# fallenshock/SinDDM

Measured on AMD Instinct MI355X. Metric: diffusion steps/sec (finest scale) + imgs/sec full multi-scale sample, 1/2/4/8 GPU, higher is better.
Workload: dtype f32 (3x3 convs: binary16 hi/lo split products -- Winograd-domain GEMMs with all 4 MFMA terms, fp32 accumulate; fp32-equivalent, error vs float64 = the fp32 oracle's: tests/test_gpu_h2.py; everything else fp32); 1 GPU; C3: 6-scale pyramid, T=1000, finest scale 411x512, batch 64 per GPU, dim=160; batch_per_gpu=64, global_batch=64, scale=5, parallelism=independent chains over 1 GPU(s), one all-gather of the images

## Files before the change

### include/sinddm_hip_debug.h

```cpp
#ifndef SINDDM_HIP_DEBUG_H
#define SINDDM_HIP_DEBUG_H

#include <stddef.h>
#include <stdint.h>

#ifdef __cplusplus
extern "C" {
#endif

int sinddm_prof_begin(void);
int sinddm_prof_end(double* conv_ms_total, int64_t* conv_launches, double* conv_flops_total);
int sinddm_prof_end2(double* conv_ms_total, int64_t* conv_launches, double* conv_flops_total,
                     double* conv_exec_flops_total);
int sinddm_prof_end3(int kind, double* ms_total, int64_t* launches, double* flops_total,
                     double* exec_flops_total, int reset);

int sinddm_debug_routes(int dim_arg, int train, int B, int H, int W, int out[16]);

int sinddm_debug_conv_path(int dim, int B, int H, int W);

int sinddm_debug_infer_path(int dim, int B, int H, int W);

int sinddm_debug_head_path(int dim, int B, int H, int W);
int sinddm_debug_head_offsets(int dim, int64_t out[3]);
int sinddm_debug_head(const float* packed, const float* g, const float* x_in, float* eps_out, int dim, int B, int H, int W,
                      int Wp, void* stream);

int sinddm_debug_train_path(int dim, int B, int H, int W);

int sinddm_debug_block_train(const float* params, const float* packed, const float* packed_bwd, int dim, int l,
                             const float* x, const float* cond_bias, const float* grad_y, float* y, float* grad_x,
                             float* grad_params, float* dcond, int B, int H, int W, void* ws, size_t ws_bytes,
                             void* stream);

int sinddm_debug_wgrad_map(int Cin, int Cout, int64_t ntiles, int ncu, uint32_t* wg_out, int wg_cap, int32_t* splits_out,
                           int splits_cap);

#define SINDDM_DWGRAD_TILES 6
#define SINDDM_DWGRAD_ROWS 7
int sinddm_debug_wgrad_plan(int taps, int Cin, int Cout, int B, int H, int W, int have_scr, int have_amax, int ncu, int out[4]);
int sinddm_debug_wgrad(int taps, int Cin, int Cout, int B, int H, int W, int ncu, int have_scr, int use_amax, const float* dout,
                       const float* in, float* gw, float* gb, void* scratch, size_t scratch_bytes, int plan_out[4], void* stream);
size_t sinddm_debug_wgrad_scratch_bytes(int taps, int Cin, int Cout, int B);
int sinddm_debug_wgrad_routes(int dim_arg, int B, int H, int W, int ncu, int* out, int cap);
// ... 6 lines not shown
```

### sinddm_amd/_lib.py

```python
from __future__ import annotations

import ctypes as C
import os
from typing import Optional

import torch

_HERE = os.path.dirname(os.path.abspath(__file__))
LIB_PATH = os.path.join(_HERE, "libsinddm_hip.so")

ABI_SYMBOLS = (
    "sinddm_abi_version", "sinddm_param_count", "sinddm_param_tensors", "sinddm_param_offset",
    "sinddm_packed_count", "sinddm_workspace_bytes", "sinddm_pack_weights", "sinddm_net_forward",
    "sinddm_q_sample", "sinddm_reverse_step", "sinddm_reverse_step_edit", "sinddm_upsample_bilinear", "sinddm_prof_begin", "sinddm_prof_end", "sinddm_prof_end2", "sinddm_prof_end3", "sinddm_debug_wgrad_map", "sinddm_debug_conv_path",
    "sinddm_debug_block_train", "sinddm_debug_infer_path", "sinddm_debug_train_path",
    "sinddm_train_workspace_bytes", "sinddm_packed_bwd_count", "sinddm_pack_weights_bwd",
    "sinddm_net_forward_train", "sinddm_net_backward", "sinddm_l1_loss_fwd_bwd", "sinddm_adam_ema_step",
    "sinddm_cond_embed", "sinddm_cond_stride", "sinddm_sample_chain", "sinddm_sample_chain2", "sinddm_sample_chain_ex",
    "sinddm_normal_fill", "sinddm_wrap_halo", "sinddm_upsample_bilinear_wrap", "sinddm_sample_chain_tile",
    "sinddm_sample_chain_keep", "sinddm_reverse_step_keep", "sinddm_normal_fill_samples", "sinddm_sample_chain_seeds",
    "sinddm_debug_head_path", "sinddm_debug_head_offsets", "sinddm_debug_head", "sinddm_debug_routes",
    "sinddm_debug_wgrad_routes", "sinddm_debug_wgrad_plan", "sinddm_debug_wgrad", "sinddm_debug_wgrad_scratch_bytes",
    "sinddm_sample_chain_resample", "sinddm_reverse_step_jump",
    "sinddm_sample_chain_layout", "sinddm_layout_delta", "sinddm_reverse_step_layout",
    "sinddm_sample_chain_batch",
    "sinddm_sample_chain_solver", "sinddm_reverse_step_ms",
    "sinddm_q_sample_wrap", "sinddm_l1_loss_crop_fwd_bwd",
    "sinddm_sample_chain_mix", "sinddm_normal_fill_mix",
    "sinddm_l1_loss_weighted_fwd_bwd",
)


ABI_VERSION = 3
DIM_FP32_CONVS = 0x10000
JUMP_STREAM = 1 << 31
MIX_MAX = 4
TILE_HALO = 16


class StepCoefs(C.Structure):
    _fields_ = [("mode", C.c_int), ("clip", C.c_int),
                ("sqrt_recip_ac_t", C.c_float), ("sqrt_recipm1_ac_t", C.c_float),
                ("coef1_t", C.c_float), ("coef2_t", C.c_float),
                ("gamma_t", C.c_float), ("gamma_tm1", C.c_float),
# ... 108 lines not shown
        "sinddm_prof_end": (i, [C.POINTER(C.c_double), C.POINTER(C.c_int64), C.POINTER(C.c_double)]),
        "sinddm_prof_end2": (i, [C.POINTER(C.c_double), C.POINTER(C.c_int64), C.POINTER(C.c_double),
                                 C.POINTER(C.c_double)]),
        "sinddm_prof_end3": (i, [i, C.POINTER(C.c_double), C.POINTER(C.c_int64), C.POINTER(C.c_double),
                                 C.POINTER(C.c_double), i]),
        "sinddm_debug_wgrad_map": (i, [i, i, i64, i, C.POINTER(C.c_uint32), i, C.POINTER(C.c_int32), i]),
        "sinddm_debug_conv_path": (i, [i, i, i, i]),
        "sinddm_debug_infer_path": (i, [i, i, i, i]),
        "sinddm_debug_train_path": (i, [i, i, i, i]),
        "sinddm_debug_head_path": (i, [i, i, i, i]),
        "sinddm_debug_routes": (i, [i, i, i, i, i, C.POINTER(C.c_int)]),
        "sinddm_debug_wgrad_routes": (i, [i, i, i, i, i, C.POINTER(C.c_int), i]),
        "sinddm_debug_wgrad_plan": (i, [i, i, i, i, i, i, i, i, i, C.POINTER(C.c_int)]),
        "sinddm_debug_wgrad": (i, [i, i, i, i, i, i, i, i, i, p, p, p, p, p, sz, C.POINTER(C.c_int), p]),
        "sinddm_debug_wgrad_scratch_bytes": (sz, [i, i, i, i]),
        "sinddm_debug_head_offsets": (i, [i, C.POINTER(C.c_int64)]),
        "sinddm_debug_head": (i, [p, p, p, p, i, i, i, i, i, p]),
        "sinddm_debug_block_train": (i, [p, p, p, i, i, p, p, p, p, p, p, p, i, i, i, p, sz, p]),
        "sinddm_train_workspace_bytes": (sz, [i, i, i, i]),
        "sinddm_packed_bwd_count": (i64, [i]),
        "sinddm_pack_weights_bwd": (i, [p, p, i, p]),
        "sinddm_net_forward_train": (i, [p, p, p, p, i, f, p, i, i, i, i, p, sz, p]),
        "sinddm_net_backward": (i, [p, p, p, p, p, p, p, i, i, i, i, p, sz, p]),
        "sinddm_l1_loss_fwd_bwd": (i, [p, p, p, p, i64, f, p]),
        "sinddm_l1_loss_crop_fwd_bwd": (i, [p, p, p, p, i, i, i, i, i, f, p]),
        "sinddm_l1_loss_weighted_fwd_bwd": (i, [p, p, p, p, p, i, i, i, i, i, i, f, f, p]),
        "sinddm_adam_ema_step": (i, [p, p, p, p, p, f, f, f, f, f, f, f, i, i64, p]),
    }
    for name, (res, args) in sig.items():
        if not hasattr(lib, name):
# ... 32 lines not shown
```

### sinddm_amd/csrc/conv_wh.h

```cpp
#pragma once
#include <utility>
#include "split16.h"

namespace sinddm {

template <class F, int... I>
__device__ __forceinline__ void wh_static_for_impl(F&& f, std::integer_sequence<int, I...>) {
    (f(std::integral_constant<int, I>{}), ...);
}
template <int N, class F>
__device__ __forceinline__ void wh_static_for(F&& f) {
    wh_static_for_impl(f, std::make_integer_sequence<int, N>{});
}

#ifndef WH_ABL
#define WH_ABL 0
#endif
#ifndef WH_MIXLO
#define WH_MIXLO 1
#endif
#ifndef WH_NT
#define WH_NT 6
#endif
#ifdef WH_TIMING
// ... 3 lines not shown
#define WH_SEG(slot) do {} while (0)
#endif
constexpr int WH_TH = 8, WH_TW = 32;
constexpr int WH_RS = 40;
constexpr int WH_PS = 408;
constexpr int WH_RAW = 16 * WH_PS * 4;
constexpr int WH_V = 24 * 2 * 64 * 16;
constexpr int WH_XS = 36;
constexpr int WH_X = 2 * 6 * 32 * WH_XS * 4;
constexpr int WH_LDS = 160 * 1024;
constexpr int WH_REGION = WH_LDS - WH_RAW;
constexpr int WH_VB = WH_REGION - WH_V;
static_assert(WH_X <= WH_VB && WH_V + WH_X <= WH_REGION && WH_VB % 16 == 0, "exchange buffer beside either V buffer");
constexpr int WH_TARGET_EXP = 10;
constexpr int WH_COB = 80;

inline bool wh_shape_ok(int cin, int cout) { return cin >= 32 && cin % 16 == 0 && cout % WH_COB == 0; }
inline long long wh_image_halfs(int cin, int cout) { return (long long)(cout / WH_COB) * (cin / 16) * 24 * 5 * 512; }

__device__ __forceinline__ int wh_shift_for(float m, int target) {
    const unsigned bits = __float_as_uint(m) & 0x7fffffffu;
    const int e = (int)(bits >> 23);
    if (e == 0 || e == 255) return 0;
    int s = target - (e - 127);
    return s > 100 ? 100 : (s < -100 ? -100 : s);
}

__device__ __forceinline__ void wh_u24(const float* __restrict__ w, long long base, int transpose, double (&u)[24]) {
    const double G2[4][3] = {{1., 0., 0.}, {.5, .5, .5}, {.5, -.5, .5}, {0., 0., 1.}};
    const double G4[6][3] = {{1. / 4, 0., 0.}, {-1. / 6, -1. / 6, -1. / 6}, {-1. / 6, 1. / 6, -1. / 6},
// ... 84 lines not shown
    hipLaunchKernelGGL(wh_pack_kernel, dim3((unsigned)((total + 255) / 256)), dim3(256), 0, st, w, wsinv,
                       static_cast<_Float16*>(img), cin, cout, transpose, total);
    SINDDM_LAUNCH_CHECK();
    return 0;
}

__device__ __forceinline__ void wh_barrier() { asm volatile("s_waitcnt lgkmcnt(0)\n\ts_barrier" ::: "memory"); }

__device__ __forceinline__ float wh_dpp_shr2(float old, float src) {
    return __builtin_bit_cast(float, __builtin_amdgcn_update_dpp(__builtin_bit_cast(int, old), __builtin_bit_cast(int, src), 0x112, 0xf, 0xf, false));
}
__device__ __forceinline__ float wh_dpp_shl2(float old, float src) {
    return __builtin_bit_cast(float, __builtin_amdgcn_update_dpp(__builtin_bit_cast(int, old), __builtin_bit_cast(int, src), 0x102, 0xf, 0xf, false));
}

__global__ __launch_bounds__(512) void conv_wh_kernel(ConvArgs p, int items_per_xcd, int wg_per_xcd) {
    typedef __attribute__((address_space(3))) float lds_f;
    extern __shared__ __attribute__((aligned(16))) float smem[];
    unsigned char* const sbytes = reinterpret_cast<unsigned char*>(smem);
    unsigned char* const sRaw = sbytes;
    unsigned char* const sV = sbytes + WH_RAW;
    const unsigned lds0 = (unsigned)(size_t)(lds_f*)smem;

    const int tid = threadIdx.x;
    const int lane = tid & 63;
    const int wv = __builtin_amdgcn_readfirstlane(tid >> 6);
    const int l16 = lane & 15, kq = lane >> 4;
    const int H = p.H, W = p.W;
    const int HW = H * W;
    const int Wt = p.Wt > 0 ? p.Wt : W;
    const int nch = p.nch3;
// ... 134 lines not shown
#else
                        const f32x2 rem{__builtin_fmaf(v[j].x, sxv, -(float)hi[pr][j].x), __builtin_fmaf(v[j].y, sxv, -(float)hi[pr][j].y)};
                        lo[pr][j] = __builtin_convertvector(rem, h16x2);
#endif
                    }
                }
#pragma unroll
                for (int j = 0; j < 6; ++j) {
                    using h16x4 = __attribute__((ext_vector_type(4))) _Float16;
                    *reinterpret_cast<h16x4*>(wp + (i * 6 + j) * 2048) = h16x4{hi[0][j][0], hi[0][j][1], hi[1][j][0], hi[1][j][1]};
                    *reinterpret_cast<h16x4*>(wp + (i * 6 + j) * 2048 + 512) = h16x4{lo[0][j][0], lo[0][j][1], lo[1][j][0], lo[1][j][1]};
                }
            });
        };

        f32x4 acc[4][2][5];
#pragma unroll
        for (int a = 0; a < 4; ++a)
#pragma unroll
            for (int g = 0; g < 2; ++g)
#pragma unroll
                for (int n = 0; n < 5; ++n) acc[a][g][n] = f32x4{0.f, 0.f, 0.f, 0.f};
        const __amdgpu_buffer_rsrc_t rsw =
            __builtin_amdgcn_make_buffer_rsrc(const_cast<float*>(p.w3), 0, 0x7FFFFFF0, 0x00020000);
        const int wlane = lane * 16;
        const int wbase = ((cb * nch) * 24 + fj) * 5 * 1024;
        h16x8 ur[10];
        auto load_u = [&](int c, int fi, int n, int slot) {
            const int so = wbase + (c * 24 * 5 + fi * 30 + n) * 1024;
            ur[slot] = __builtin_bit_cast(h16x8, __builtin_amdgcn_raw_buffer_load_b128(rsw, wlane, so, 0));
        };
        auto multiply = [&](int c, const unsigned char* vb) {
            const unsigned char* A = vb + fj * 2048 + a_rd;
            wh_static_for<4>([&](auto FI) {
                constexpr int fi = decltype(FI)::value;
                constexpr int fo = fi * 6 * 2048;
                h16x8 ah0, ah1, al0, al1;
                ah0 = *reinterpret_cast<const h16x8*>(A + fo);
                ah1 = *reinterpret_cast<const h16x8*>(A + fo + 1024);
                al0 = *reinterpret_cast<const h16x8*>(A + fo + 512);
                al1 = *reinterpret_cast<const h16x8*>(A + fo + 1024 + 512);
                wh_static_for<5>([&](auto NN) {
                    constexpr int n = decltype(NN)::value;
                    constexpr int slot = (fi & 1) * 5 + n;
                    const h16x8 u = ur[slot];
                    __builtin_amdgcn_sched_barrier(0);
                    if (WH_ABL & 8) {
// ... 2 lines not shown
                        acc[fi][0][n] = __builtin_amdgcn_mfma_f32_16x16x32_f16(al0, u, acc[fi][0][n], 0, 0, 0);
                        acc[fi][1][n] = __builtin_amdgcn_mfma_f32_16x16x32_f16(al1, u, acc[fi][1][n], 0, 0, 0);
                        acc[fi][0][n] = __builtin_amdgcn_mfma_f32_16x16x32_f16(ah0, u, acc[fi][0][n], 0, 0, 0);
                        acc[fi][1][n] = __builtin_amdgcn_mfma_f32_16x16x32_f16(ah1, u, acc[fi][1][n], 0, 0, 0);
                    }
                    __builtin_amdgcn_sched_barrier(0);
                    if (!(WH_ABL & 4)) {
                        if (fi < 2) load_u(c, fi + 2, n, slot);
                        else load_u(c + 1 < nch ? c + 1 : c, fi - 2, n, slot);
                    }
                    __builtin_amdgcn_sched_barrier(0);
                });
            });
        };

        const int e_t = tid & 31, e_co = tid >> 5;
        const int e_tr = e_t >> 3, e_tc = e_t & 7;
        const int ey = y0 + 2 * e_tr, ex = x0 + 4 * e_tc;
        f32x4 rsd[5][2];
        float ek[5], ebv[5];
        auto ep_operands = [&]() {
            const bool e_in = ex < W;
#pragma unroll
            for (int n = 0; n < 5; ++n) {
                const int co = cb * WH_COB + n * 16 + e_co;
                ek[n] = inv_sx * p.wsinv[co];
                ebv[n] = p.bias ? p.bias[co] : 0.0f;
#pragma unroll
                for (int pp = 0; pp < 2; ++pp) {
                    rsd[n][pp] = f32x4{0.f, 0.f, 0.f, 0.f};
                    if (p.resid && !(WH_ABL & 16) && e_in && ey + pp < H)
                        rsd[n][pp] = ((WH_NT & 2) && big_out) ? __builtin_nontemporal_load(reinterpret_cast<const f32x4*>(p.resid + ((size_t)b * p.Cout + co) * HW + (size_t)(ey + pp) * W + ex))
                                                 : *reinterpret_cast<const f32x4*>(p.resid + ((size_t)b * p.Cout + co) * HW + (size_t)(ey + pp) * W + ex);
                }
            }
        };

        WH_SEG(0);
        if constexpr (service) {
            const __amdgpu_buffer_rsrc_t rsnx = in_rsrc(nxt.ok ? nxt.b : b);
            float sxn = 0.f, inv_n = 0.f;
            if (nxt.ok) item_scale(nxt, sxn, inv_n);
            if (j == 0) {
                stage_write(sRaw);
                if (nch > 1) stage_load(rsin, svoff, 1);
                else if (nxt.ok) { stage_offsets(nxt, svoff); stage_load(rsnx, svoff, 0); }
                WH_SEG(1);
                transform(sRaw, vbuf(g), sx);
                wh_barrier();
            }
            WH_SEG(2);
            for (int c = 0; c < nch; ++c) {
                if (c + 1 < nch || nxt.ok) {
                    stage_write(sRaw);
                    if (c + 2 < nch) stage_load(rsin, svoff, c + 2);
                    else if (nxt.ok) {
                        if (c + 2 == nch) stage_offsets(nxt, svoff);
                        if (c + 2 == nch || nch > 1) stage_load(rsnx, svoff, c + 2 - nch);
                    }
                    if (c == 3) WH_SEG(24);
                    transform(sRaw, vbuf(g + c + 1), c + 1 < nch ? sx : sxn);
                    if (c == 3) WH_SEG(25);
                }
                wh_barrier();
                if (c < 12) WH_SEG(3 + c);
            }
            ep_operands();
        } else {
            wh_static_for<10>([&](auto SL) {
                constexpr int sl = decltype(SL)::value;
                load_u(0, sl / 5, sl % 5, sl);
            });
            WH_SEG(1);
            if (j == 0) wh_barrier();
            WH_SEG(2);
            for (int c = 0; c < nch; ++c) {
                multiply(c, vbuf(g + c));
                if (c == 3) WH_SEG(25);
                wh_barrier();
                if (c < 12) WH_SEG(3 + c);
            }
            ep_operands();
        }
        g += nch;
        WH_SEG(16);

        const int e_wr = ((fj * 32 + l16) * WH_XS + 4 * kq) * 4;
        const int e_rd = (e_co * WH_XS + e_t) * 4;
        float amax = 0.f;
        WH_SEG(17);
        if constexpr (!service) {
#pragma unroll
            for (int mg = 0; mg < 2; ++mg)
#pragma unroll
                for (int n = 0; n < 5; ++n) {
                    acc[0][mg][n] = acc[0][mg][n] + acc[1][mg][n] + acc[2][mg][n];
                    acc[1][mg][n] = acc[1][mg][n] - acc[2][mg][n] - acc[3][mg][n];
                }
        }
        wh_static_for<3>([&](auto PS) {
            constexpr int n0 = 2 * decltype(PS)::value;
            constexpr int nn = n0 + 2 <= 5 ? 2 : 1;
            unsigned char* X = sV + ((g & 1) ? 0 : WH_V);
            if constexpr (!service) {
#pragma unroll
                for (int r = 0; r < 2; ++r)
#pragma unroll
                    for (int nl = 0; nl < nn; ++nl)
#pragma unroll
                        for (int mg = 0; mg < 2; ++mg)
                            *reinterpret_cast<f32x4*>(X + e_wr + (r * 6 * 32 + nl * 16) * (WH_XS * 4) + mg * 64) = acc[r][mg][n0 + nl];
            }
            wh_barrier();
            WH_SEG(18 + decltype(PS)::value);
            float q[nn][2][6];
#pragma unroll
            for (int nl = 0; nl < nn; ++nl)
#pragma unroll
                for (int r = 0; r < 2; ++r)
#pragma unroll
                    for (int j = 0; j < 6; ++j)
                        q[nl][r][j] = *reinterpret_cast<const float*>(X + e_rd + ((r * 6 + j) * 32 + nl * 16) * (WH_XS * 4));
            wh_barrier();
            wh_static_for<nn>([&](auto NL) {
                constexpr int n = n0 + decltype(NL)::value;
                const int co = cb * WH_COB + n * 16 + e_co;
                const float k = ek[n];
                const float bv = ebv[n];
#pragma unroll
                for (int pp = 0; pp < 2; ++pp) {
                    const float* z = q[decltype(NL)::value][pp];
                    const float s12 = z[1] + z[2], d12 = z[1] - z[2], s34 = z[3] + z[4], d34 = z[3] - z[4];
                    f32x4 v{z[0] + s12 + s34, d12 + 2.f * d34, s12 + 4.f * s34, d12 + 8.f * d34 + z[5]};
                    const int y = ey + pp;
                    if ((WH_ABL & 16) && v[0] != 123.456f) continue;
                    if (y < H && ex < W) {
                        const size_t o = ((size_t)b * p.Cout + co) * HW + (size_t)y * W + ex;
                        v = v * k + bv;
                        if (p.out_pre) *reinterpret_cast<f32x4*>(p.out_pre + o) = v;
                        if (p.act == 1) v = gelu_erf4(v);
                        else if (p.act == 2) {
// ... 12 lines not shown
                        else *reinterpret_cast<f32x4*>(p.out + o) = v;
                    }
                }
            });
        });
        if (p.amax_out) amax_publish(amax, p.amax_out + (size_t)b * AMAX_STRIDE);
        WH_SEG(23);
        if (!nxt.ok) break;
        cur = nxt;
    }
    };
    if (service_rt) role_body(std::true_type{});
    else role_body(std::false_type{});
}

#ifndef SINDDM_WH_MIN_ITEMS_PER_CU
#define SINDDM_WH_MIN_ITEMS_PER_CU 12
#endif
#ifndef SINDDM_WH_MIN_PIXELS
#define SINDDM_WH_MIN_PIXELS 12000
#endif
#ifndef SINDDM_CONV_WH
#define SINDDM_CONV_WH 1
#endif
inline bool conv_wh_applies(bool fp32_convs, int B, int H, int W, int cin, int cout) {
    if (!SINDDM_CONV_WH || fp32_convs || !wh_shape_ok(cin, cout) || W % 4 != 0) return false;
    if ((long long)cin * H * W * 4 >= 0x40000000LL) return false;
    if ((long long)H * W < SINDDM_WH_MIN_PIXELS) return false;
    return (long long)B * ((W + WH_TW - 1) / WH_TW) * ((H + WH_TH - 1) / WH_TH) * (cout / WH_COB) >=
           (long long)SINDDM_WH_MIN_ITEMS_PER_CU * cu_count();
}

inline int conv_wh_launch(const ConvArgs& a_in, hipStream_t st) {
    ConvArgs a = a_in;
    if (!wh_shape_ok(a.Cin, a.Cout) || a.W % 4 != 0 || !a.wsinv || (long long)a.Cin * a.H * a.W * 4 >= 0x40000000LL)
        return SINDDM_E_BADSHAPE;
    ConvProfiler& prof = conv_profiler();
    const bool rec = prof.begin(st);
    a.nch3 = a.Cin / 16;
    a.coblks = a.Cout / WH_COB;
    a.tilesX = (a.W + WH_TW - 1) / WH_TW;
    a.tilesY = (a.H + WH_TH - 1) / WH_TH;
    a.ntiles = a.B * a.tilesX * a.tilesY;
    a.tiles_per_xcd = (a.ntiles + 7) / 8;
    const int ipx = a.tiles_per_xcd * a.coblks;
    int wpx = cu_count() / 8;
    if (wpx < 1) wpx = 1;
    if (wpx > ipx) wpx = ipx;
    static const hipError_t attr_rc = hipFuncSetAttribute(reinterpret_cast<const void*>(&conv_wh_kernel),
                                                          hipFuncAttributeMaxDynamicSharedMemorySize, WH_LDS);
    if (attr_rc != hipSuccess) return (int)attr_rc;
#ifdef WH_TIMING
    static int wh_launch_no = 0;
    a.mtp = wh_launch_no++ % 8;
#endif
    hipLaunchKernelGGL(conv_wh_kernel, dim3(wpx * 8), dim3(512), WH_LDS, st, a, ipx, wpx);
    if (rec) {
        const double fl = 2.0 * a.B * a.H * (a.Wt > 0 ? a.Wt : a.W) * (double)a.Cout * 9.0 * a.Cin;
        prof.end(st, 1, fl, 2.0 * a.ntiles * 32.0 * 24.0 * 4.0 * (double)a.Cout * a.Cin, 8);
    }
    SINDDM_LAUNCH_CHECK();
    return 0;
}

}
```

### sinddm_amd/csrc/internal.h

```cpp
#pragma once
#include "common.h"

namespace sinddm {

struct PackSeg {
    long long dst;
    long long count;
    long long w;
    long long w2;
    int kind;
    int cin, cout, taps, nch, mt, co_lds;
    int transpose;
};
struct PackArgs {
    PackSeg seg[32];
    int nseg;
    long long total;
};
int pack_launch(const float* params, float* packed, const PackArgs& a, hipStream_t st);

inline void pack_add_direct(PackArgs& a, long long dst, long long w, int cin, int cout, int taps, int mt, int coblks, int transpose) {
    PackSeg s{};
    s.kind = 0; s.transpose = transpose; s.w2 = -1;
    s.dst = dst; s.w = w; s.cin = cin; s.cout = cout; s.taps = taps; s.mt = mt; s.co_lds = co_lds_for(mt);
// ... 35 lines not shown
    float* wscr;
    float* amax;
};

struct ChainStep;
int net_forward_impl(const NetPlan& P, const float* params, const float* packed, const float* x, const int64_t* t_dev,
                     int t_host, float scale, float* out, int B, int H, int W, void* ws, size_t ws_bytes,
                     hipStream_t st, const TrainBufs* tb, const ChainStep* cs = nullptr);

int block_forward(const NetPlan& P, int l, const float* params, const float* packed, const float* cur, const float* cond,
                  int cond_stride, float* hbuf, float* gbuf, float* obuf, float* upre, int B, int H, int W, hipStream_t st,
                  const int route[2], int Wt = 0, float* amax = nullptr);
enum ConvKernel { CONV_DIRECT = 0, CONV_C3 = 1, CONV_WINO2 = 2, CONV_WINO3 = 3, CONV_WINO4 = 4, CONV_WH = 8 };
ConvKernel conv3x3_route(const NetPlan& P, const Conv3x3Images& c, int B, int H, int W, bool have_amax, bool first_conv);
struct ConvArgs;
int conv3x3_launch(ConvKernel k, const Conv3x3Images& c, const float* packed, ConvArgs a, hipStream_t st);
bool forward_routes(const NetPlan& P, bool train, int B, int H, int Wp, bool have_amax, int out[8]);
int forward_pitch(const NetPlan& P, int W);

bool wh_enabled();
int wh_pack(const Conv3x3Images& c, const float* w, float* packed, int transpose, hipStream_t st);
int amax_tensor_launch(const float* x, float* amax, int B, long long per_sample, hipStream_t st);

int dwconv_launch(const float* x, const float* w, const float* bias, const float* cond, int cond_stride,
                  const float* addt, int flip, float* out, int B, int C, int H, int W, hipStream_t st, int pi = 0, int po = 0,
                  float* amax = nullptr);

}
```

### sinddm_amd/csrc/sinddm_bwd.hip

```cpp
#include <utility>
#include "conv_args.h"
#include "conv1x1.h"
#include "internal.h"
#include "wgrad_plan.h"
#include "wgrad_wh.h"

namespace sinddm {

struct WgradArgs {
    const float* dout;
    const float* in;
    const float* zero;
    float* gw;
    float* gb;
    int B, H, W, Cin, Cout;
    int coblks, ciblks, S;
    int tilesX, tilesY, ntiles;
    int abl;
    int scr;
};

template <int MT, int TAPS>
__global__ __launch_bounds__(WG_THREADS, 2) void wgrad_mfma_kernel(WgradArgs p) {
    typedef __attribute__((address_space(3))) void* lds_ptr;
// ... 966 lines not shown
        rc = amax_tensor_launch(dO, amax_b + 2 * l, B, (long long)b.cout * H * W, st);
        if (rc) return rc;
    }
    rc = wgrad_launch(d.w2, zp, dO, tb.g[l], grads + b.c2_w, grads + b.c2_b, st, tb.wscr, d.wh2 ? amax_b + 2 * l : nullptr,
                      d.wh2 ? tb.amax + 2 * l + 1 : nullptr);
    if (rc) return rc;
    if (d.wres.nwg > 0) {
        rc = wgrad_launch(d.wres, zp, dO, xin, grads + b.res_w, grads + b.res_b, st);
        if (rc) return rc;
    }
    {
        ConvArgs c{};
        c.zero = zp; c.in = dO; c.Cin = b.cout; c.aux = tb.u[l]; c.act = 2; c.out = dU; c.Cout = b.cout;
        c.B = B; c.H = H; c.W = W;
        if (d.wh2) { c.amax_in = amax_b + 2 * l; c.amax_out = d.wh1 ? amax_b + 2 * l + 1 : nullptr; }
        rc = conv3x3_launch(d.dg2, k.dg2[l], packed_bwd, c, st);
    }
    if (rc) return rc;
    rc = wgrad_launch(d.w1, zp, dU, tb.h[l], grads + b.c1_w, grads + b.c1_b, st, tb.wscr, d.wha ? amax_b + 2 * l + 1 : nullptr,
                      d.wha ? tb.amax + 2 * l : nullptr);
    if (rc) return rc;
    {
        ConvArgs c{};
        c.zero = zp; c.in = dU; c.Cin = b.cout; c.act = 0; c.out = dH; c.Cout = b.cin;
        c.B = B; c.H = H; c.W = W;
        if (d.wh1) c.amax_in = amax_b + 2 * l + 1;
        rc = conv3x3_launch(d.dg1, k.dg1[l], packed_bwd, c, st);
    }
    if (rc) return rc;
    hipLaunchKernelGGL(d.dw_rows ? dwconv5_wgrad_rows_kernel : dwconv5_wgrad_kernel, dim3(b.cin, B), dim3(256), 0, st, dH, xin,
                       grads + b.dw_w, grads + b.dw_b, tb.dcond + b.cond_off, P.cond_stride, b.cin, H, W);
    SINDDM_LAUNCH_CHECK();
    if (dst) {
        const float* radd = dO;
        if (b.res_w >= 0) {
            rc = conv1x1_dgrad(zp, dO, b.cout, packed_bwd + k.dres[l], conv3x3_nch(k.dg1[l]), dU, b.cin, k.dg1[l].mt,
                               k.dg1[l].coblks, B, H, W, st);
            if (rc) return rc;
            radd = dU;
        }
        rc = dwconv_launch(dH, params + b.dw_w, nullptr, nullptr, 0, radd, 1, dst, B, b.cin, H, W, st, 0, 0,
                           d.pub ? amax_b + 2 * (l - 1) : nullptr);
// ... 309 lines not shown
```

### sinddm_amd/csrc/sinddm_fwd.hip

```cpp
#include "conv_mfma.h"
#include "conv_wino4.h"
#include "conv_wh.h"
#include "internal.h"
#include "step_tail.h"
#include "chain_run.h"
#include <type_traits>
namespace sinddm {

ConvProfiler& conv_profiler() {
    static ConvProfiler p;
    return p;
}

__global__ void pack_kernel(const float* __restrict__ params, float* __restrict__ packed, PackArgs a) {
    long long i = (long long)blockIdx.x * blockDim.x + threadIdx.x;
    if (i >= a.total) return;
    int s = 0;
    long long base = 0;
    while (s < a.nseg - 1 && i >= base + a.seg[s].count) { base += a.seg[s].count; ++s; }
    const PackSeg& g = a.seg[s];
    const long long j = i - base;
    float v = 0.0f;
    if (g.kind == 0) {
        const int co_l = (int)(j % g.co_lds);
// ... 813 lines not shown
static HeadEps head_eps(const NetPlan& P, const float* packed, const float* g, const float* xin, int H, int Wp) {
    return HeadEps{g, xin, packed + P.pk_hc, packed + P.pk_hr, packed + P.pk_hb, P.half, P.dim, H, Wp};
}

ConvKernel conv3x3_route(const NetPlan& P, const Conv3x3Images& c, int B, int H, int W, bool have_amax, bool first_conv) {
    if (wino_enabled() && c.K % 4 == 0) {
        if (have_amax && c.wh >= 0 && conv_wh_applies(P.fp32_convs, B, H, W, c.K, c.M)) return CONV_WH;
        if (SINDDM_WINO_V3 && c.wino24 >= 0 &&
            (long long)B * ((W + 31) / 32) * ((H + 3) / 4) * c.coblks >= SINDDM_V3_MIN_ITEMS_PER_CU * cu_count())
            return SINDDM_WINO_V4 && conv_wino4_applies(B, H, W, c.coblks) ? CONV_WINO4 : CONV_WINO3;
        if (c.wino2 >= 0) return CONV_WINO2;
    }
    return first_conv && c.K == 3 && SINDDM_CONV_C3 ? CONV_C3 : CONV_DIRECT;
}

int conv3x3_launch(ConvKernel k, const Conv3x3Images& c, const float* packed, ConvArgs a, hipStream_t st) {
    a.coblks = c.coblks;
    switch (k) {
        case CONV_WH:
            a.w3 = packed + c.wh; a.wsinv = packed + c.wh_sinv;
            return conv_wh_launch(a, st);
        case CONV_WINO4:
        case CONV_WINO3:
            a.w3 = packed + c.wino24; a.nch3 = conv3x3_nchw(c);
            return k == CONV_WINO4 ? conv_wino4_launch(a, st) : conv_wino3_launch(a, st);
        case CONV_WINO2:
            if (a.Cin % 4 != 0) return SINDDM_E_BADSHAPE;
            a.w3 = packed + c.wino2; a.nch3 = conv3x3_nchw(c);
            return conv_wino2_launch(a, c.mt, st);
        case CONV_DIRECT:
            a.w3 = packed + c.direct; a.nch3 = conv3x3_nch(c);
            return conv_launch(a, c.mt, st);
        default: return SINDDM_E_BADARG;
    }
}

// ... 3 lines not shown
    for (int l = 0; l < 4; ++l) {
        out[2 * l] = conv3x3_route(P, P.blk[l].c1, B, H, Wp, have_amax, true);
        out[2 * l + 1] = head && l == 3 ? -1 : conv3x3_route(P, P.blk[l].c2, B, H, Wp, have_amax, false);
        any = any || out[2 * l] == CONV_WH || out[2 * l + 1] == CONV_WH;
    }
    return any;
}
int forward_pitch(const NetPlan& P, int W) { return fwd_pitch(P, W); }

int block_forward(const NetPlan& P, int l, const float* params, const float* packed, const float* cur, const float* cond,
                  int cond_stride, float* hbuf, float* gbuf, float* obuf, float* upre, int B, int H, int W, hipStream_t st,
                  const int route[2], int Wt, float* amax) {
    const BlockPlan& b = P.blk[l];
    const bool wha = route[0] == CONV_WH, whb = route[1] == CONV_WH;
    if ((wha || whb) && !amax) return SINDDM_E_BADARG;
    int rc = Wt > 0 ? dwconv_launch(cur, params + b.dw_w, params + b.dw_b, cond, cond_stride, nullptr, 0, hbuf, B, b.cin, H,
                                    Wt, st, W, W, wha ? amax : nullptr)
                    : dwconv_launch(cur, params + b.dw_w, params + b.dw_b, cond, cond_stride, nullptr, 0, hbuf, B, b.cin, H,
                                    W, st, 0, 0, wha ? amax : nullptr);
    if (rc) return rc;
    if (route[0] == CONV_C3) {
        const int nwg = ((H * W + 255) / 256) * B;
        int split = 1;
        while (split < 8 && nwg * split < 2048 && b.cout % (split * 2) == 0) split *= 2;
        hipLaunchKernelGGL(conv3x3_c3_gelu_kernel, dim3((H * W + 255) / 256, B, split), dim3(256), 0, st, hbuf,
                           params + b.c1_w, params + b.c1_b, gbuf, upre, H, W, b.cout, b.cout / split, Wt > 0 ? Wt : W,
                           whb ? amax + 1 : nullptr);
        SINDDM_LAUNCH_CHECK();
    } else {
        ConvArgs c1{};
        c1.in = hbuf; c1.out = gbuf; c1.out_pre = upre;
        c1.B = B; c1.H = H; c1.W = W; c1.Cin = b.cin; c1.Cout = b.cout;
        c1.act = 1; c1.zero = packed + P.pk_zero; c1.Wt = Wt;
        c1.bias = wha ? params + b.c1_b : packed + b.pk_b1;
        if (wha) { c1.amax_in = amax; c1.amax_out = whb ? amax + 1 : nullptr; }
        rc = conv3x3_launch((ConvKernel)route[0], b.c1, packed, c1, st);
    }
    if (rc || route[1] < 0) return rc;
    if (whb && !wha && route[0] != CONV_C3) {
        rc = amax_tensor_launch(gbuf, amax + 1, B, (long long)b.cout * H * W, st);
        if (rc) return rc;
    }
    ConvArgs c2{};
    c2.in = gbuf; c2.out = obuf;
    c2.B = B; c2.H = H; c2.W = W; c2.Cin = b.cout; c2.Cout = b.cout;
    c2.act = 0; c2.zero = packed + P.pk_zero; c2.Wt = Wt;
    c2.bias = packed + b.pk_b2;
    if (b.nchr == 0) c2.resid = cur;
    else if (route[1] == CONV_DIRECT) {
        c2.in2 = cur; c2.Cin2 = b.cin; c2.w1 = packed + b.pk_res; c2.nch1 = b.nchr;
    } else {
        ConvArgs r1{};
        r1.in2 = cur; r1.Cin2 = b.cin; r1.w1 = packed + b.pk_res; r1.nch1 = b.nchr; r1.nch3 = 0;
        r1.bias = packed + b.pk_b2; r1.out = obuf; r1.Cout = b.cout; r1.coblks = b.coblks;
        r1.B = B; r1.H = H; r1.W = W; r1.zero = packed + P.pk_zero;
        rc = conv1x1_launch(r1, b.mt, st);
        if (rc) return rc;
        c2.resid = obuf; c2.bias = nullptr;
    }
    if (whb) c2.amax_in = amax + 1;
    return conv3x3_launch((ConvKernel)route[1], b.c2, packed, c2, st);
}

bool wh_enabled() { return SINDDM_CONV_WH != 0; }
int wh_pack(const Conv3x3Images& c, const float* w, float* packed, int transpose, hipStream_t st) {
    if (c.wh < 0) return 0;
    return wh_pack_launch(w, packed + c.wh_sinv, packed + c.wh, transpose ? c.M : c.K, transpose ? c.K : c.M, transpose, st);
}

__global__ __launch_bounds__(256) void amax_tensor_kernel(const float* __restrict__ x, float* __restrict__ amax, long long n4) {
    const int b = blockIdx.y;
    const f32x4* p = reinterpret_cast<const f32x4*>(x) + (size_t)b * n4;
    float m = 0.f;
    for (long long i = (long long)blockIdx.x * 256 + threadIdx.x; i < n4; i += (long long)gridDim.x * 256) {
        const f32x4 v = p[i];
        m = fmaxf(m, fmaxf(fmaxf(fabsf(v.x), fabsf(v.y)), fmaxf(fabsf(v.z), fabsf(v.w))));
// ... 815 lines not shown
    return 0;
}

int sinddm_debug_head(const float* packed, const float* g, const float* x_in, float* eps_out, int dim, int B, int H, int W,
                      int Wp, void* stream) {
    if (!packed || !g || !x_in || !eps_out || B <= 0 || H <= 0 || W <= 0) return SINDDM_E_BADARG;
    NetPlan p = make_plan(dim);
    if (!p.ok) return SINDDM_E_BADSHAPE;
    if (Wp % 4 != 0 || W > Wp || W <= Wp - 4 || (long long)H * Wp >= (1LL << 28) || B > 65535) return SINDDM_E_BADSHAPE;
    hipLaunchKernelGGL(head_eps_kernel, dim3((unsigned)((H * (Wp / 4) + 255) / 256), B), dim3(256), 0,
                       static_cast<hipStream_t>(stream), head_eps(p, packed, g, x_in, H, Wp), eps_out, W);
    SINDDM_LAUNCH_CHECK();
    return 0;
}

int sinddm_prof_end3(int kind, double* ms_total, int64_t* launches, double* flops_total, double* exec_flops_total,
                     int reset) {
    ConvProfiler& p = conv_profiler();
    p.on = false;
    double ms = 0.0, fl = 0.0, ex = 0.0;
    int64_t n = 0;
    for (int i = 0; i < p.used; ++i) {
        if (kind >= 10 ? (p.kind[i] != kind / 10 || p.gen[i] != kind % 10) : (kind != 0 && p.kind[i] != kind)) continue;
        hipError_t e = hipEventSynchronize(p.ev[2 * i + 1]);
        if (e != hipSuccess) return (int)e;
        float t = 0.f;
        e = hipEventElapsedTime(&t, p.ev[2 * i], p.ev[2 * i + 1]);
        if (e != hipSuccess) return (int)e;
        ms += t; fl += p.rec_flops[i]; ex += p.rec_exec[i]; ++n;
    }
// ... 39 lines not shown
```

Before: 769.6 sample-steps/s (finest scale, batch x steps/s, all GPUs).

## Add wide-Cout Winograd conv variant with 160-channel blocks and ring-buffered weight loads

Adds a templated conv_wr_kernel that processes 160 output channels per work item (10 column tiles, 2 accumulator rows) instead of 80. It reuses each loaded Winograd-domain activation fragment across twice as many output channels, and streams weight fragments through a 4-slot register ring with prefetch. Epilogue operand loads are interleaved with the exchange stages. Inference routes to it by default when Cout is divisible by 160 and there are enough items per CU, while training and backward keep the old kernel. The cost is higher register pressure, which could reduce occupancy, and fewer work items for load balancing.

```diff
diff --git a/include/sinddm_hip_debug.h b/include/sinddm_hip_debug.h
--- a/include/sinddm_hip_debug.h
+++ b/include/sinddm_hip_debug.h
@@ -28,6 +28,11 @@
 
 int sinddm_debug_train_path(int dim, int B, int H, int W);
 
+int sinddm_debug_conv_wh(int variant, int ncu, int B, int H, int W, int Wt, int Cin, int Cout, int act, const float* in,
+                         const float* weights, const float* bias, const float* resid, const float* aux, float* out,
+                         float* out_pre, float* amax_out, void* scratch, size_t scratch_bytes, void* stream);
+size_t sinddm_debug_conv_wh_scratch_bytes(int Cin, int Cout, int B);
+
 int sinddm_debug_block_train(const float* params, const float* packed, const float* packed_bwd, int dim, int l,
                              const float* x, const float* cond_bias, const float* grad_y, float* y, float* grad_x,
                              float* grad_params, float* dcond, int B, int H, int W, void* ws, size_t ws_bytes,
diff --git a/sinddm_amd/_lib.py b/sinddm_amd/_lib.py
--- a/sinddm_amd/_lib.py
+++ b/sinddm_amd/_lib.py
@@ -28,6 +28,7 @@
     "sinddm_q_sample_wrap", "sinddm_l1_loss_crop_fwd_bwd",
     "sinddm_sample_chain_mix", "sinddm_normal_fill_mix",
     "sinddm_l1_loss_weighted_fwd_bwd",
+    "sinddm_debug_conv_wh", "sinddm_debug_conv_wh_scratch_bytes",
 )
 
 
@@ -166,6 +167,8 @@
         "sinddm_debug_wgrad_plan": (i, [i, i, i, i, i, i, i, i, i, C.POINTER(C.c_int)]),
         "sinddm_debug_wgrad": (i, [i, i, i, i, i, i, i, i, i, p, p, p, p, p, sz, C.POINTER(C.c_int), p]),
         "sinddm_debug_wgrad_scratch_bytes": (sz, [i, i, i, i]),
+        "sinddm_debug_conv_wh": (i, [i, i, i, i, i, i, i, i, i, p, p, p, p, p, p, p, p, p, sz, p]),
+        "sinddm_debug_conv_wh_scratch_bytes": (sz, [i, i, i]),
         "sinddm_debug_head_offsets": (i, [i, C.POINTER(C.c_int64)]),
         "sinddm_debug_head": (i, [p, p, p, p, i, i, i, i, i, p]),
         "sinddm_debug_block_train": (i, [p, p, p, i, i, p, p, p, p, p, p, p, i, i, i, p, sz, p]),
diff --git a/sinddm_amd/csrc/conv_wh.h b/sinddm_amd/csrc/conv_wh.h
--- a/sinddm_amd/csrc/conv_wh.h
+++ b/sinddm_amd/csrc/conv_wh.h
@@ -41,6 +41,8 @@
 static_assert(WH_X <= WH_VB && WH_V + WH_X <= WH_REGION && WH_VB % 16 == 0, "exchange buffer beside either V buffer");
 constexpr int WH_TARGET_EXP = 10;
 constexpr int WH_COB = 80;
+constexpr int WR_RING = 4;
+static_assert(40 % WR_RING == 0 && WR_RING <= 10, "static ring slots");
 
 inline bool wh_shape_ok(int cin, int cout) { return cin >= 32 && cin % 16 == 0 && cout % WH_COB == 0; }
 inline long long wh_image_halfs(int cin, int cout) { return (long long)(cout / WH_COB) * (cin / 16) * 24 * 5 * 512; }
@@ -155,7 +157,10 @@
     return __builtin_bit_cast(float, __builtin_amdgcn_update_dpp(__builtin_bit_cast(int, old), __builtin_bit_cast(int, src), 0x102, 0xf, 0xf, false));
 }
 
-__global__ __launch_bounds__(512) void conv_wh_kernel(ConvArgs p, int items_per_xcd, int wg_per_xcd) {
+template <bool WR>
+__device__ __forceinline__ void wh_run(const ConvArgs& p, int items_per_xcd, int wg_per_xcd) {
+    constexpr int NCT = WR ? 10 : 5;
+    constexpr int NROW = WR ? 2 : 4;
     typedef __attribute__((address_space(3))) float lds_f;
     extern __shared__ __attribute__((aligned(16))) float smem[];
     unsigned char* const sbytes = reinterpret_cast<unsigned char*>(smem);
@@ -320,23 +325,54 @@
             });
         };
 
-        f32x4 acc[4][2][5];
-#pragma unroll
-        for (int a = 0; a < 4; ++a)
+        f32x4 acc[NROW][2][NCT];
+#pragma unroll
+        for (int a = 0; a < NROW; ++a)
 #pragma unroll
             for (int g = 0; g < 2; ++g)
 #pragma unroll
-                for (int n = 0; n < 5; ++n) acc[a][g][n] = f32x4{0.f, 0.f, 0.f, 0.f};
+                for (int n = 0; n < NCT; ++n) acc[a][g][n] = f32x4{0.f, 0.f, 0.f, 0.f};
         const __amdgpu_buffer_rsrc_t rsw =
             __builtin_amdgcn_make_buffer_rsrc(const_cast<float*>(p.w3), 0, 0x7FFFFFF0, 0x00020000);
         const int wlane = lane * 16;
-        const int wbase = ((cb * nch) * 24 + fj) * 5 * 1024;
+        const int wbase = (((WR ? 2 : 1) * cb * nch) * 24 + fj) * 5 * 1024;
+        const int wcb = nch * 24 * 5 * 1024;
         h16x8 ur[10];
         auto load_u = [&](int c, int fi, int n, int slot) {
-            const int so = wbase + (c * 24 * 5 + fi * 30 + n) * 1024;
+            const int so = wbase + (c * 24 * 5 + fi * 30 + (WR ? n % 5 : n)) * 1024 + (WR && n >= 5 ? wcb : 0);
             ur[slot] = __builtin_bit_cast(h16x8, __builtin_amdgcn_raw_buffer_load_b128(rsw, wlane, so, 0));
         };
-        auto multiply = [&](int c, const unsigned char* vb) {
+        auto multiply_wr = [&](auto c, const unsigned char* vb) {
+            const unsigned char* A = vb + fj * 2048 + a_rd;
+            wh_static_for<4>([&](auto FI) {
+                constexpr int fi = decltype(FI)::value;
+                constexpr int fo = fi * 6 * 2048;
+                h16x8 ah0, ah1, al0, al1;
+                ah0 = *reinterpret_cast<const h16x8*>(A + fo);
+                ah1 = *reinterpret_cast<const h16x8*>(A + fo + 1024);
+                al0 = *reinterpret_cast<const h16x8*>(A + fo + 512);
+                al1 = *reinterpret_cast<const h16x8*>(A + fo + 1024 + 512);
+                wh_static_for<10>([&](auto NN) {
+                    constexpr int n = decltype(NN)::value;
+                    constexpr int q = fi * 10 + n, slot = q % WR_RING, qn = (q + WR_RING) % 40;
+                    const h16x8 u = ur[slot];
+                    const f32x4 zero{0.f, 0.f, 0.f, 0.f};
+                    __builtin_amdgcn_sched_barrier(0);
+                    f32x4 q0 = __builtin_amdgcn_mfma_f32_16x16x32_f16(al0, u, zero, 0, 0, 0);
+                    f32x4 q1 = __builtin_amdgcn_mfma_f32_16x16x32_f16(al1, u, zero, 0, 0, 0);
+                    q0 = __builtin_amdgcn_mfma_f32_16x16x32_f16(ah0, u, q0, 0, 0, 0);
+                    q1 = __builtin_amdgcn_mfma_f32_16x16x32_f16(ah1, u, q1, 0, 0, 0);
+                    __builtin_amdgcn_sched_barrier(0);
+                    if (q + WR_RING < 40) load_u(c, qn / 10, qn % 10, slot);
+                    else load_u(c + 1 < nch ? c + 1 : c, qn / 10, qn % 10, slot);
+                    __builtin_amdgcn_sched_barrier(0);
+                    if constexpr (fi < 3) { acc[0][0][n] += q0; acc[0][1][n] += q1; }
+                    if constexpr (fi == 1) { acc[1][0][n] += q0; acc[1][1][n] += q1; }
+                    if constexpr (fi >= 2) { acc[1][0][n] -= q0; acc[1][1][n] -= q1; }
+                });
+            });
+        };
+        auto multiply = [&](auto c, const unsigned char* vb) {
             const unsigned char* A = vb + fj * 2048 + a_rd;
             wh_static_for<4>([&](auto FI) {
                 constexpr int fi = decltype(FI)::value;
@@ -369,16 +405,22 @@
             });
         };
 
-        const int e_t = tid & 31, e_co = tid >> 5;
-        const int e_tr = e_t >> 3, e_tc = e_t & 7;
-        const int ey = y0 + 2 * e_tr, ex = x0 + 4 * e_tc;
-        f32x4 rsd[5][2];
-        float ek[5], ebv[5];
-        auto ep_operands = [&]() {
+        int e_t, e_co, ey, ex;
+        auto ep_thread = [&]() {
+            int t = tid;
+            if constexpr (WR) asm volatile("" : "+v"(t));
+            e_t = t & 31; e_co = t >> 5;
+            const int e_tr = e_t >> 3, e_tc = e_t & 7;
+            ey = y0 + 2 * e_tr; ex = x0 + 4 * e_tc;
+        };
+        if constexpr (!WR) ep_thread();
+        f32x4 rsd[NCT][2];
+        float ek[NCT], ebv[NCT];
+        auto ep_operands = [&](auto N0, auto N1) {
             const bool e_in = ex < W;
 #pragma unroll
-            for (int n = 0; n < 5; ++n) {
-                const int co = cb * WH_COB + n * 16 + e_co;
+            for (int n = decltype(N0)::value; n < decltype(N1)::value; ++n) {
+                const int co = cb * (NCT * 16) + n * 16 + e_co;
                 ek[n] = inv_sx * p.wsinv[co];
                 ebv[n] = p.bias ? p.bias[co] : 0.0f;
 #pragma unroll
@@ -390,6 +432,8 @@
                 }
             }
         };
+        constexpr std::integral_constant<int, 0> ep_n0{};
+        constexpr std::integral_constant<int, WR ? 2 : 5> ep_n1{};
 
         WH_SEG(0);
         if constexpr (service) {
@@ -420,31 +464,37 @@
                 wh_barrier();
                 if (c < 12) WH_SEG(3 + c);
             }
-            ep_operands();
+            if constexpr (WR) ep_thread();
+            ep_operands(ep_n0, ep_n1);
         } else {
             wh_static_for<10>([&](auto SL) {
                 constexpr int sl = decltype(SL)::value;
-                load_u(0, sl / 5, sl % 5, sl);
+                if constexpr (!WR) load_u(0, sl / 5, sl % 5, sl);
+                else if constexpr (sl < WR_RING) load_u(0, 0, sl, sl);
             });
             WH_SEG(1);
             if (j == 0) wh_barrier();
             WH_SEG(2);
             for (int c = 0; c < nch; ++c) {
-                multiply(c, vbuf(g + c));
+                if constexpr (WR) multiply_wr(c, vbuf(g + c));
+                else multiply(c, vbuf(g + c));
                 if (c == 3) WH_SEG(25);
                 wh_barrier();
                 if (c < 12) WH_SEG(3 + c);
             }
-            ep_operands();
+            if constexpr (WR) ep_thread();
+            ep_operands(ep_n0, ep_n1);
         }
         g += nch;
         WH_SEG(16);
 
-        const int e_wr = ((fj * 32 + l16) * WH_XS + 4 * kq) * 4;
+        int e_lane = lane;
+        if constexpr (WR) asm volatile("" : "+v"(e_lane));
+        const int e_wr = ((fj * 32 + (e_lane & 15)) * WH_XS + 4 * (e_lane >> 4)) * 4;
         const int e_rd = (e_co * WH_XS + e_t) * 4;
         float amax = 0.f;
         WH_SEG(17);
-        if constexpr (!service) {
+        if constexpr (!service && !WR) {
 #pragma unroll
             for (int mg = 0; mg < 2; ++mg)
 #pragma unroll
@@ -453,9 +503,9 @@
                     acc[1][mg][n] = acc[1][mg][n] - acc[2][mg][n] - acc[3][mg][n];
                 }
         }
-        wh_static_for<3>([&](auto PS) {
+        wh_static_for<(NCT + 1) / 2>([&](auto PS) {
             constexpr int n0 = 2 * decltype(PS)::value;
-            constexpr int nn = n0 + 2 <= 5 ? 2 : 1;
+            constexpr int nn = n0 + 2 <= NCT ? 2 : 1;
             unsigned char* X = sV + ((g & 1) ? 0 : WH_V);
             if constexpr (!service) {
 #pragma unroll
@@ -466,6 +516,8 @@
                         for (int mg = 0; mg < 2; ++mg)
                             *reinterpret_cast<f32x4*>(X + e_wr + (r * 6 * 32 + nl * 16) * (WH_XS * 4) + mg * 64) = acc[r][mg][n0 + nl];
             }
+            if constexpr (WR && n0 + 2 < NCT)
+                ep_operands(std::integral_constant<int, n0 + 2>{}, std::integral_constant<int, n0 + 4>{});
             wh_barrier();
             WH_SEG(18 + decltype(PS)::value);
             float q[nn][2][6];
@@ -479,7 +531,7 @@
             wh_barrier();
             wh_static_for<nn>([&](auto NL) {
                 constexpr int n = n0 + decltype(NL)::value;
-                const int co = cb * WH_COB + n * 16 + e_co;
+                const int co = cb * (NCT * 16) + n * 16 + e_co;
                 const float k = ek[n];
                 const float bv = ebv[n];
 #pragma unroll
@@ -522,6 +574,13 @@
     else role_body(std::false_type{});
 }
 
+__global__ __launch_bounds__(512) void conv_wh_kernel(ConvArgs p, int items_per_xcd, int wg_per_xcd) {
+    wh_run<false>(p, items_per_xcd, wg_per_xcd);
+}
+__global__ __launch_bounds__(512) void conv_wr_kernel(ConvArgs p, int items_per_xcd, int wg_per_xcd) {
+    wh_run<true>(p, items_per_xcd, wg_per_xcd);
+}
+
 #ifndef SINDDM_WH_MIN_ITEMS_PER_CU
 #define SINDDM_WH_MIN_ITEMS_PER_CU 12
 #endif
@@ -539,30 +598,50 @@
            (long long)SINDDM_WH_MIN_ITEMS_PER_CU * cu_count();
 }
 
-inline int conv_wh_launch(const ConvArgs& a_in, hipStream_t st) {
+#ifndef SINDDM_CONV_WR
+#define SINDDM_CONV_WR 1
+#endif
+constexpr int WR_COB = 2 * WH_COB;
+#ifndef SINDDM_WR_MIN_ITEMS_PER_CU
+#define SINDDM_WR_MIN_ITEMS_PER_CU 12
+#endif
+
+inline bool conv_wr_pays(int B, int H, int W, int cout) {
+    if (!SINDDM_CONV_WR || cout % WR_COB != 0) return false;
+    return (long long)B * ((W + WH_TW - 1) / WH_TW) * ((H + WH_TH - 1) / WH_TH) * (cout / WR_COB) >=
+           (long long)SINDDM_WR_MIN_ITEMS_PER_CU * cu_count();
+}
+
+inline int conv_wh_launch(const ConvArgs& a_in, hipStream_t st, int variant = 0, int ncu = 0) {
     ConvArgs a = a_in;
     if (!wh_shape_ok(a.Cin, a.Cout) || a.W % 4 != 0 || !a.wsinv || (long long)a.Cin * a.H * a.W * 4 >= 0x40000000LL)
         return SINDDM_E_BADSHAPE;
+    if (variant < 0 || variant > 2) return SINDDM_E_BADARG;
+    if (variant == 2 && a.Cout % WR_COB != 0) return SINDDM_E_BADSHAPE;
+    const bool wr = variant == 2 || (variant == 0 && SINDDM_CONV_WR && a.Cout % WR_COB == 0);
     ConvProfiler& prof = conv_profiler();
     const bool rec = prof.begin(st);
     a.nch3 = a.Cin / 16;
-    a.coblks = a.Cout / WH_COB;
+    a.coblks = a.Cout / (wr ? WR_COB : WH_COB);
     a.tilesX = (a.W + WH_TW - 1) / WH_TW;
     a.tilesY = (a.H + WH_TH - 1) / WH_TH;
     a.ntiles = a.B * a.tilesX * a.tilesY;
     a.tiles_per_xcd = (a.ntiles + 7) / 8;
     const int ipx = a.tiles_per_xcd * a.coblks;
-    int wpx = cu_count() / 8;
+    int wpx = (ncu > 0 ? ncu : cu_count()) / 8;
     if (wpx < 1) wpx = 1;
     if (wpx > ipx) wpx = ipx;
     static const hipError_t attr_rc = hipFuncSetAttribute(reinterpret_cast<const void*>(&conv_wh_kernel),
                                                           hipFuncAttributeMaxDynamicSharedMemorySize, WH_LDS);
+    static const hipError_t attr_rc_wr = hipFuncSetAttribute(reinterpret_cast<const void*>(&conv_wr_kernel),
+                                                             hipFuncAttributeMaxDynamicSharedMemorySize, WH_LDS);
     if (attr_rc != hipSuccess) return (int)attr_rc;
+    if (attr_rc_wr != hipSuccess) return (int)attr_rc_wr;
 #ifdef WH_TIMING
     static int wh_launch_no = 0;
     a.mtp = wh_launch_no++ % 8;
 #endif
-    hipLaunchKernelGGL(conv_wh_kernel, dim3(wpx * 8), dim3(512), WH_LDS, st, a, ipx, wpx);
+    hipLaunchKernelGGL(wr ? conv_wr_kernel : conv_wh_kernel, dim3(wpx * 8), dim3(512), WH_LDS, st, a, ipx, wpx);
     if (rec) {
         const double fl = 2.0 * a.B * a.H * (a.Wt > 0 ? a.Wt : a.W) * (double)a.Cout * 9.0 * a.Cin;
         prof.end(st, 1, fl, 2.0 * a.ntiles * 32.0 * 24.0 * 4.0 * (double)a.Cout * a.Cin, 8);
diff --git a/sinddm_amd/csrc/internal.h b/sinddm_amd/csrc/internal.h
--- a/sinddm_amd/csrc/internal.h
+++ b/sinddm_amd/csrc/internal.h
@@ -73,7 +73,7 @@
 enum ConvKernel { CONV_DIRECT = 0, CONV_C3 = 1, CONV_WINO2 = 2, CONV_WINO3 = 3, CONV_WINO4 = 4, CONV_WH = 8 };
 ConvKernel conv3x3_route(const NetPlan& P, const Conv3x3Images& c, int B, int H, int W, bool have_amax, bool first_conv);
 struct ConvArgs;
-int conv3x3_launch(ConvKernel k, const Conv3x3Images& c, const float* packed, ConvArgs a, hipStream_t st);
+int conv3x3_launch(ConvKernel k, const Conv3x3Images& c, const float* packed, ConvArgs a, hipStream_t st, int wh_variant = 0);
 bool forward_routes(const NetPlan& P, bool train, int B, int H, int Wp, bool have_amax, int out[8]);
 int forward_pitch(const NetPlan& P, int W);
 
diff --git a/sinddm_amd/csrc/sinddm_bwd.hip b/sinddm_amd/csrc/sinddm_bwd.hip
--- a/sinddm_amd/csrc/sinddm_bwd.hip
+++ b/sinddm_amd/csrc/sinddm_bwd.hip
@@ -1004,7 +1004,7 @@
         c.zero = zp; c.in = dO; c.Cin = b.cout; c.aux = tb.u[l]; c.act = 2; c.out = dU; c.Cout = b.cout;
         c.B = B; c.H = H; c.W = W;
         if (d.wh2) { c.amax_in = amax_b + 2 * l; c.amax_out = d.wh1 ? amax_b + 2 * l + 1 : nullptr; }
-        rc = conv3x3_launch(d.dg2, k.dg2[l], packed_bwd, c, st);
+        rc = conv3x3_launch(d.dg2, k.dg2[l], packed_bwd, c, st, 1);
     }
     if (rc) return rc;
     rc = wgrad_launch(d.w1, zp, dU, tb.h[l], grads + b.c1_w, grads + b.c1_b, st, tb.wscr, d.wha ? amax_b + 2 * l + 1 : nullptr,
@@ -1015,7 +1015,7 @@
         c.zero = zp; c.in = dU; c.Cin = b.cout; c.act = 0; c.out = dH; c.Cout = b.cin;
         c.B = B; c.H = H; c.W = W;
         if (d.wh1) c.amax_in = amax_b + 2 * l + 1;
-        rc = conv3x3_launch(d.dg1, k.dg1[l], packed_bwd, c, st);
+        rc = conv3x3_launch(d.dg1, k.dg1[l], packed_bwd, c, st, 1);
     }
     if (rc) return rc;
     hipLaunchKernelGGL(d.dw_rows ? dwconv5_wgrad_rows_kernel : dwconv5_wgrad_kernel, dim3(b.cin, B), dim3(256), 0, st, dH, xin,
diff --git a/sinddm_amd/csrc/sinddm_fwd.hip b/sinddm_amd/csrc/sinddm_fwd.hip
--- a/sinddm_amd/csrc/sinddm_fwd.hip
+++ b/sinddm_amd/csrc/sinddm_fwd.hip
@@ -851,12 +851,13 @@
     return first_conv && c.K == 3 && SINDDM_CONV_C3 ? CONV_C3 : CONV_DIRECT;
 }
 
-int conv3x3_launch(ConvKernel k, const Conv3x3Images& c, const float* packed, ConvArgs a, hipStream_t st) {
+int conv3x3_launch(ConvKernel k, const Conv3x3Images& c, const float* packed, ConvArgs a, hipStream_t st, int wh_variant) {
     a.coblks = c.coblks;
     switch (k) {
         case CONV_WH:
             a.w3 = packed + c.wh; a.wsinv = packed + c.wh_sinv;
-            return conv_wh_launch(a, st);
+            if (wh_variant == 0 && !conv_wr_pays(a.B, a.H, a.W, a.Cout)) wh_variant = 1;
+            return conv_wh_launch(a, st, wh_variant);
         case CONV_WINO4:
         case CONV_WINO3:
             a.w3 = packed + c.wino24; a.nch3 = conv3x3_nchw(c);
@@ -890,6 +891,7 @@
     const BlockPlan& b = P.blk[l];
     const bool wha = route[0] == CONV_WH, whb = route[1] == CONV_WH;
     if ((wha || whb) && !amax) return SINDDM_E_BADARG;
+    const int wh_variant = upre ? 1 : 0;
     int rc = Wt > 0 ? dwconv_launch(cur, params + b.dw_w, params + b.dw_b, cond, cond_stride, nullptr, 0, hbuf, B, b.cin, H,
                                     Wt, st, W, W, wha ? amax : nullptr)
                     : dwconv_launch(cur, params + b.dw_w, params + b.dw_b, cond, cond_stride, nullptr, 0, hbuf, B, b.cin, H,
@@ -910,7 +912,7 @@
         c1.act = 1; c1.zero = packed + P.pk_zero; c1.Wt = Wt;
         c1.bias = wha ? params + b.c1_b : packed + b.pk_b1;
         if (wha) { c1.amax_in = amax; c1.amax_out = whb ? amax + 1 : nullptr; }
-        rc = conv3x3_launch((ConvKernel)route[0], b.c1, packed, c1, st);
+        rc = conv3x3_launch((ConvKernel)route[0], b.c1, packed, c1, st, wh_variant);
     }
     if (rc || route[1] < 0) return rc;
     if (whb && !wha && route[0] != CONV_C3) {
@@ -935,7 +937,7 @@
         c2.resid = obuf; c2.bias = nullptr;
     }
     if (whb) c2.amax_in = amax + 1;
-    return conv3x3_launch((ConvKernel)route[1], b.c2, packed, c2, st);
+    return conv3x3_launch((ConvKernel)route[1], b.c2, packed, c2, st, wh_variant);
 }
 
 bool wh_enabled() { return SINDDM_CONV_WH != 0; }
@@ -1781,6 +1783,47 @@
     return 0;
 }
 
+static size_t wh_debug_round(size_t v) { return (v + 255) / 256 * 256; }
+static bool wh_debug_shape_ok(int Cin, int Cout, int B) { return B >= 1 && B <= 65535 && Cin >= 32 && Cin % 16 == 0 && Cout >= 80 && Cout % 80 == 0; }
+
+size_t sinddm_debug_conv_wh_scratch_bytes(int Cin, int Cout, int B) {
+    if (!wh_debug_shape_ok(Cin, Cout, B)) return 0;
+    return wh_debug_round((size_t)wh_image_halfs(Cin, Cout) * 2) + wh_debug_round((size_t)Cout * sizeof(float)) +
+           wh_debug_round((size_t)B * AMAX_STRIDE * sizeof(float));
+}
+
+int sinddm_debug_conv_wh(int variant, int ncu, int B, int H, int W, int Wt, int Cin, int Cout, int act, const float* in,
+                         const float* weights, const float* bias, const float* resid, const float* aux, float* out,
+                         float* out_pre, float* amax_out, void* scratch, size_t scratch_bytes, void* stream) {
+    if (!in || !weights || !out || !scratch || (act == 2 && !aux)) return SINDDM_E_BADARG;
+    if (variant < 0 || variant > 2 || act < 0 || act > 2 || B <= 0 || H <= 0 || W <= 0 || Cin <= 0 || Cout <= 0)
+        return SINDDM_E_BADARG;
+    if (W % 4 != 0 || !wh_debug_shape_ok(Cin, Cout, B) || (variant == 2 && Cout % 160 != 0)) return SINDDM_E_BADSHAPE;
+    if (Wt != 0 && (Wt > W || Wt <= W - 4)) return SINDDM_E_BADSHAPE;
+    if ((long long)Cin * H * W * 4 >= 0x40000000LL || (long long)B * ((H + 7) / 8) * ((W + 31) / 32) > 0x3fffffffLL)
+        return SINDDM_E_BADSHAPE;
+    if (scratch_bytes < sinddm_debug_conv_wh_scratch_bytes(Cin, Cout, B) || (uintptr_t)scratch % 256 != 0) return SINDDM_E_BADARG;
+    for (const void* q : {(const void*)in, (const void*)resid, (const void*)aux, (const void*)out, (const void*)out_pre})
+        if ((uintptr_t)q % 16 != 0) return SINDDM_E_BADARG;
+
+    hipStream_t st = static_cast<hipStream_t>(stream);
+    char* base = static_cast<char*>(scratch);
+    void* img = base;
+    float* wsinv = reinterpret_cast<float*>(base + wh_debug_round((size_t)wh_image_halfs(Cin, Cout) * 2));
+    float* amax_in = wsinv + wh_debug_round((size_t)Cout * sizeof(float)) / sizeof(float);
+    int rc = wh_pack_launch(weights, wsinv, img, Cin, Cout, 0, st);
+    if (rc) return rc;
+    const hipError_t e = hipMemsetAsync(amax_in, 0, (size_t)B * AMAX_STRIDE * sizeof(float), st);
+    if (e != hipSuccess) return (int)e;
+    rc = amax_tensor_launch(in, amax_in, B, (long long)Cin * H * W, st);
+    if (rc) return rc;
+    ConvArgs a{};
+    a.in = in; a.resid = resid; a.aux = aux; a.bias = bias; a.out = out; a.out_pre = out_pre;
+    a.w3 = static_cast<const float*>(img); a.wsinv = wsinv; a.amax_in = amax_in; a.amax_out = amax_out;
+    a.B = B; a.H = H; a.W = W; a.Cin = Cin; a.Cout = Cout; a.act = act; a.Wt = Wt;
+    return conv_wh_launch(a, st, variant, ncu);
+}
+
 int sinddm_prof_end3(int kind, double* ms_total, int64_t* launches, double* flops_total, double* exec_flops_total,
                      int reset) {
     ConvProfiler& p = conv_profiler();
```

Result: faster. 804.3 sample-steps/s (finest scale, batch x steps/s, all GPUs) (median of 6 runs) (+4.5%).
